# zhangganlin/vista-slam

Hardware: AMD Instinct MI355X
Metric: STA image-pairs/sec @512x384 (higher is better)
Workload: dtype f16x3-split MFMA (3 fp16 products) in the transformer and the pose head; fp16 MFMA + one block-scaled fp8 correction MFMA in the DPT head's convolutions; fp32 accumulate; 1 GPU; 512x384 batch=8 pairs/GPU STA two-view forward (BASELINE configs[1]); pairs_per_gpu=8, H=384, W=512, precision=f16x3h, parallelism=single GPU

## Files before the change

include/sta_mi355_debug.h:

```cpp
#ifndef STA_MI355_DEBUG_H
#define STA_MI355_DEBUG_H
#include "sta_mi355.h"
#ifdef __cplusplus
extern "C" {
#endif

STA_API int sta_set_gemm_variant(sta_handle* h, int variant);

STA_API int sta_debug_pick_family(int amode, int epi, long long M, int N, int K, int split, int cstride, int Ho, int Wo);

STA_API int sta_debug_gemm_plan(int amode, int epi, int M_all, int N, int K, int precision, int mx, int tail_hint, int forced_variant, int* out);

STA_API int sta_debug_last_gemm_plan(sta_handle* h, int* out);

STA_API int sta_debug_qkv_pair_plan(int precision, int M, int N_a, int N_b, int K, int mx_a, int mx_b, int tail_hint, int forced_variant, int* out);

STA_API int sta_debug_qkv_pair(sta_handle* h, const float* x_a, const float* w_a, const float* bias_a, const float* x_b,
                       const float* w_b, const float* bias_b, int S, int ntok, int K, int C, int wp,
                       float* q_a, float* k_a, float* vt_a, float* k_b, float* vt_b, void* stream);

STA_API int sta_debug_gemm(sta_handle* h, const float* A, const float* W, const float* bias, int M, int N, int K,
                   int act, int via_f16, const float* resid, float* out, void* stream);

STA_API int sta_debug_qkv_rope(sta_handle* h, const float* x, const float* W, const float* bias, int S, int ntok, int K, int C,
// ... 22 lines not shown

STA_API int sta_debug_head_final(sta_handle* h, const float* x, const float* w, const float* bias, int64_t npix,
                         float* pts, float* conf, void* stream);

STA_API int sta_debug_svd_orthogonalize(sta_handle* h, const float* m, float* r, int B, void* stream);

STA_API int sta_kernel_timing_dump(sta_handle* h, int cap, double* flops, float* ms, int* variant, int* n_out);

STA_API int sta_kernel_stamps_dump(sta_handle* h, int cap, double* out6, int* n_out);

STA_API int sta_bench_gemm_stamps(sta_handle* h, int M, int N, int K, int resid, double* out, unsigned long long* raw_host, int raw_cap, void* stream);

STA_API int sta_bench_gemm(sta_handle* h, int M, int N, int K, int iters, int tile, int ablation, float* ms_out, void* stream);
STA_API float sta_bench_gemm_last_ghz(void);
STA_API int sta_bench_attention(sta_handle* h, int S, int heads, int nq, int nk, int pose, int iters, int which, float* ms_out, void* stream);

#ifdef __cplusplus
}
#endif
#endif
```

vista_slam_amd/_lib.py:

```python
import ctypes as C
import os

PKG = os.path.dirname(os.path.abspath(__file__))
LIB_PATH = os.path.join(PKG, "libsta_mi355.so")
TEST_LIB_PATH = os.path.join(PKG, "libsta_mi355_test.so")

STA_PREC_F16 = 1
STA_PREC_F16X3 = 3
STA_PREC_F16X3H = 5
STA_PREC_F16X3M = 6
PRECISIONS = {"f16": STA_PREC_F16, "f16x3": STA_PREC_F16X3, "f16x3h": STA_PREC_F16X3H, "f16x3m": STA_PREC_F16X3M}


class StaConfig(C.Structure):
    _fields_ = [("patch_size", C.c_int32), ("enc_embed_dim", C.c_int32), ("enc_depth", C.c_int32),
                ("enc_num_heads", C.c_int32), ("dec_embed_dim", C.c_int32), ("dec_depth", C.c_int32),
                ("dec_num_heads", C.c_int32), ("mlp_ratio", C.c_int32), ("rope_base", C.c_float),
                ("ln_eps", C.c_float), ("precision", C.c_int32)]


_vp, _i, _i64, _f = C.c_void_p, C.c_int, C.c_int64, C.c_float
_fp = C.c_void_p

SIGNATURES = {
# ... 46 lines not shown
    "sta_kernel_timing_filter": (_i, [_vp, _i, _i, _i, _i, _i]),
    "sta_kernel_timing_dump_shapes": (_i, [_vp, _i, C.POINTER(_i), C.POINTER(C.c_float), C.POINTER(_i), C.POINTER(_i)]),
    "sta_range_report": (_i, [_vp, C.POINTER(C.c_ulonglong), _i]),
    "sta_last_error": (C.c_char_p, []),
    "sta_version": (C.c_char_p, []),
}

TEST_SIGNATURES = {
    "sta_set_gemm_variant": (_i, [_vp, _i]),
    "sta_kernel_timing_dump": (_i, [_vp, _i, C.POINTER(C.c_double), C.POINTER(C.c_float), C.POINTER(_i), C.POINTER(_i)]),
    "sta_kernel_stamps_dump": (_i, [_vp, _i, C.POINTER(C.c_double), C.POINTER(_i)]),
    "sta_bench_gemm_stamps": (_i, [_vp, _i, _i, _i, _i, C.POINTER(C.c_double), C.POINTER(C.c_ulonglong), _i, _vp]),
    "sta_bench_gemm": (_i, [_vp, _i, _i, _i, _i, _i, _i, C.POINTER(_f), _vp]),
    "sta_bench_gemm_last_ghz": (C.c_float, []),
    "sta_bench_attention": (_i, [_vp, _i, _i, _i, _i, _i, _i, _i, C.POINTER(_f), _vp]),
    "sta_debug_gemm": (_i, [_vp, _fp, _fp, _fp, _i, _i, _i, _i, _i, _fp, _fp, _vp]),
    "sta_debug_qkv_rope": (_i, [_vp, _fp, _fp, _fp, _i, _i, _i, _i, _i, _i, _fp, _fp, _fp, _vp]),
    "sta_debug_attention": (_i, [_vp, _fp, _fp, _fp, _i, _i, _i, _i, _i, _fp, _vp]),
    "sta_debug_attention_pose": (_i, [_vp, _fp, _fp, _fp, _i, _i, _i, _i, _fp, _vp]),
    "sta_debug_set_tail_hint": (_i, [_vp, _i]),
    "sta_debug_set_option": (_i, [_vp, _i, _i]),
    "sta_debug_pick_family": (_i, [_i, _i, C.c_longlong, _i, _i, _i, _i, _i, _i]),
    "sta_debug_gemm_plan": (_i, [_i, _i, _i, _i, _i, _i, _i, _i, _i, C.POINTER(_i)]),
    "sta_debug_last_gemm_plan": (_i, [_vp, C.POINTER(_i)]),
    "sta_debug_qkv_pair_plan": (_i, [_i, _i, _i, _i, _i, _i, _i, _i, _i, C.POINTER(_i)]),
    "sta_debug_qkv_pair": (_i, [_vp, _fp, _fp, _fp, _fp, _fp, _fp, _i, _i, _i, _i, _i, _fp, _fp, _fp, _fp, _fp, _vp]),
    "sta_debug_conv3x3": (_i, [_vp, _fp, _fp, _fp, _i, _i, _i, _i, _i, _i, _i, _i, _fp, _fp, _vp]),
    "sta_debug_convt": (_i, [_vp, _fp, _fp, _fp, _i, _i, _i, _i, _i, _fp, _vp]),
    "sta_debug_up2": (_i, [_vp, _fp, _i, _i, _i, _i, _i, _i, _fp, _vp]),
    "sta_debug_layernorm": (_i, [_vp, _fp, _fp, _fp, _i, _i, _f, _fp, _fp, _vp]),
# ... 81 lines not shown
```

vista_slam_amd/csrc/attention.h:

```cpp
#pragma once
#include "sta_common.h"
#include <type_traits>

__device__ __forceinline__ void glds16(const void* gsrc, void* lds_dst_wave_base);

struct AttnParams {
    const f16* Q_hi; const f16* Q_lo; const f16* K_hi; const f16* K_lo; const f16* Vt_hi; const f16* Vt_lo;
    f16* O_hi; f16* O_lo; int ldo;
    int S, heads, nq, nk, npad;
    int kv_shift;
    float scale_log2e;
    unsigned long long* range;
    int prefetch;
    int pose;
};

#define ATT_KV 64
#define ATT_TILE_BYTES (64 * 128)

template <bool SPLIT>
constexpr int attn_smem_bytes(int stages = 2) { return stages * (SPLIT ? 4 : 2) * ATT_TILE_BYTES; }
#define ATT_PREFETCH_TILES 4

template <bool SPLIT>
__device__ __forceinline__ void attn_pose_query(const AttnParams& p, char* smem) {
    const int tid = threadIdx.x, lane = tid & 63, wave = tid >> 6;
    const int sh = blockIdx.x;
    const int s = sh / p.heads, h = sh - s * p.heads;
    const int skv = (s + p.kv_shift) % p.S;
    const size_t qoff = ((size_t)(s * p.heads + h) * p.npad + p.nq) * 64;
// ... 57 lines not shown
#pragma unroll
            for (int e = 0; e < 8; ++e) o = __builtin_fmaf(pe[e], (float)a[u].e[e] + (SPLIT ? (float)b[u].e[e] : 0.f), o);
        }
    }
    red[8 + wave * 64 + lane] = o;
    __syncthreads();
    if (wave != 0) return;
    o = (red[8 + lane] + red[8 + 64 + lane]) + (red[8 + 128 + lane] + red[8 + 192 + lane]);
    o /= (red[4] + red[5]) + (red[6] + red[7]);
    const int64_t orow = (int64_t)p.S * p.nq + s, orows = (int64_t)p.S * p.nq + p.S;
    const size_t oo = blk_off<SPLIT>(orow, h * 64 + lane, orows);
    if (SPLIT) { f16 hh, ll; split_f16(o, hh, ll, p.range); p.O_hi[oo] = hh; p.O_hi[oo + 32] = ll; }
    else p.O_hi[oo] = to_f16_sat(o, p.range);
}

template <bool SPLIT>
__global__ __launch_bounds__(256, 2) void attn_kernel(const AttnParams p) {
    extern __shared__ __attribute__((aligned(16))) char smem[];
    constexpr int NPL = SPLIT ? 2 : 1;
    constexpr int STAGE = 2 * NPL * ATT_TILE_BYTES;
    const int npose_blocks = p.pose == 1 ? p.S * p.heads : 0;
    const int nqe = p.nq + (p.pose == 2 ? 1 : 0);
    if ((int)blockIdx.x < npose_blocks) { attn_pose_query<SPLIT>(p, smem); return; }
    const int tid = threadIdx.x, lane = tid & 63;
    const int wave = __builtin_amdgcn_readfirstlane(tid >> 6);
    const int l31 = lane & 31, lhi = lane >> 5;
    const int nqb = (nqe + 127) / 128;
    const int nwg = nqb * p.heads * p.S;
    int logical;
    {
        const int bid = blockIdx.x - npose_blocks, q = nwg / 8, r = nwg % 8, xcd = bid % 8;
        logical = (xcd < r ? xcd * (q + 1) : r * (q + 1) + (xcd - r) * q) + bid / 8;
    }
    const int qb = logical % nqb;
    const int h = (logical / nqb) % p.heads, s = logical / (nqb * p.heads);
    const int skv = (s + p.kv_shift) % p.S;
    const int q0 = qb * 128 + wave * 32;

    const size_t qoff = (size_t)(s * p.heads + h) * p.npad * 64;
    const size_t koff = (size_t)(skv * p.heads + h) * p.npad * 64;
    const size_t voff = (size_t)(skv * p.heads + h) * 64 * p.npad;

    half8 qf_hi[4], qf_lo[4];
    {
        int qrow = q0 + l31; if (qrow > nqe - 1) qrow = nqe - 1;
        const f16* qp = p.Q_hi + qoff + (size_t)qrow * 64 + lhi * 8;
#pragma unroll
        for (int kk = 0; kk < 4; ++kk) { H8 t; t.u = ldg16(qp + kk * 16); qf_hi[kk] = t.h; }
        if (SPLIT) {
            const f16* ql = p.Q_lo + qoff + (size_t)qrow * 64 + lhi * 8;
#pragma unroll
            for (int kk = 0; kk < 4; ++kk) { H8 t; t.u = ldg16(ql + kk * 16); qf_lo[kk] = t.h; }
        }
    }

    int ksrc_l[2], vsrc_l[2];
#pragma unroll
    for (int i = 0; i < 2; ++i) {
        const int row = (2 * wave + i) * 8 + (lane >> 3);
        const int sch = (lane & 7) ^ ((row >> 1) & 7);
        ksrc_l[i] = row * 64 + sch * 8;
        vsrc_l[i] = row * p.npad + sch * 8;
    }
    auto issue_tile = [&](int stage, int kv0) {
        char* sK = smem + stage * STAGE + (2 * wave) * 1024;
        char* sV = sK + NPL * ATT_TILE_BYTES;
#pragma unroll
        for (int i = 0; i < 2; ++i) {
            const size_t ko = koff + (size_t)kv0 * 64 + ksrc_l[i];
            const size_t vo = voff + (size_t)kv0 + vsrc_l[i];
            glds16(p.K_hi + ko, sK + i * 1024);
            glds16(p.Vt_hi + vo, sV + i * 1024);
            if (SPLIT) {
                glds16(p.K_lo + ko, sK + ATT_TILE_BYTES + i * 1024);
                glds16(p.Vt_lo + vo, sV + ATT_TILE_BYTES + i * 1024);
            }
        }
    };

    floatx16 oacc[2];
#pragma unroll
    for (int d = 0; d < 2; ++d)
#pragma unroll
        for (int r = 0; r < 16; ++r) oacc[d][r] = 0.f;
    float m_run = -INFINITY, l_run = 0.f;
    const bool wave_active = q0 < nqe;

    if (p.pose && wave_active) {
        float sp = 0.f;
#pragma unroll
        for (int kk = 0; kk < 4; ++kk) {
            H8 a, b; a.u = ldg16(p.K_hi + koff + (size_t)p.nk * 64 + kk * 16 + lhi * 8);
            if (SPLIT) b.u = ldg16(p.K_lo + koff + (size_t)p.nk * 64 + kk * 16 + lhi * 8);
#pragma unroll
            for (int e = 0; e < 8; ++e) {
                const float kv = (float)a.e[e] + (SPLIT ? (float)b.e[e] : 0.f);
                const float qv = (float)qf_hi[kk][e] + (SPLIT ? (float)qf_lo[kk][e] : 0.f);
                sp = __builtin_fmaf(qv, kv, sp);
            }
        }
        sp += __shfl_xor(sp, 32);
        m_run = sp * p.scale_log2e;
        l_run = lhi == 0 ? 1.f : 0.f;
#pragma unroll
        for (int d = 0; d < 2; ++d)
#pragma unroll
            for (int r = 0; r < 16; ++r) {
                const size_t o = voff + (size_t)(d * 32 + (r & 3) + 8 * (r >> 2) + 4 * lhi) * p.npad + p.nk;
                oacc[d][r] = (float)p.Vt_hi[o] + (SPLIT ? (float)p.Vt_lo[o] : 0.f);
            }
    }

    int foff_l[4];
    {
        const int swz = (l31 >> 1) & 7;
#pragma unroll
        for (int c2 = 0; c2 < 4; ++c2) foff_l[c2] = l31 * 128 + (((c2 * 2 + lhi) ^ swz) << 4);
    }

    auto tile_body = [&](auto stage_c, auto tail_c, int kv0, int stage_rt = 0) {
        constexpr int STG = decltype(stage_c)::value;
        constexpr bool TAIL = decltype(tail_c)::value;
        const char* sK = smem + STG * STAGE + stage_rt * STAGE;
        const char* sV = sK + NPL * ATT_TILE_BYTES;

        floatx16 sacc[2];
#pragma unroll
        for (int t = 0; t < 2; ++t) {
#pragma unroll
            for (int r = 0; r < 16; ++r) sacc[t][r] = 0.f;
#pragma unroll
            for (int kk = 0; kk < 4; ++kk) {
                half8 kf = *reinterpret_cast<const half8*>(sK + t * 4096 + foff_l[kk]);
                if (SPLIT) {
                    half8 kl = *reinterpret_cast<const half8*>(sK + ATT_TILE_BYTES + t * 4096 + foff_l[kk]);
                    sacc[t] = __builtin_amdgcn_mfma_f32_32x32x16_f16(kl, qf_hi[kk], sacc[t], 0, 0, 0);
                    sacc[t] = __builtin_amdgcn_mfma_f32_32x32x16_f16(kf, qf_lo[kk], sacc[t], 0, 0, 0);
                }
                sacc[t] = __builtin_amdgcn_mfma_f32_32x32x16_f16(kf, qf_hi[kk], sacc[t], 0, 0, 0);
            }
        }

        if (TAIL) {
#pragma unroll
            for (int t = 0; t < 2; ++t)
#pragma unroll
                for (int r = 0; r < 16; ++r) {
                    const int key = kv0 + t * 32 + (r & 3) + 8 * (r >> 2) + 4 * lhi;
                    if (key >= p.nk) sacc[t][r] = -INFINITY;
                }
        }
        float mx = -INFINITY;
#pragma unroll
        for (int t = 0; t < 2; ++t)
#pragma unroll
            for (int r = 0; r < 16; ++r) mx = fmaxf(mx, sacc[t][r]);
        mx = fmaxf(mx, __shfl_xor(mx, 32));
        const float m_new = fmaxf(m_run, mx * p.scale_log2e);
        const float alpha = __builtin_amdgcn_exp2f(m_run - m_new);
        const float neg_m = -m_new;
        float psum = 0.f;
#pragma unroll
        for (int t = 0; t < 2; ++t)
#pragma unroll
            for (int r = 0; r < 16; ++r) {
                const float pv = __builtin_amdgcn_exp2f(__builtin_fmaf(sacc[t][r], p.scale_log2e, neg_m));
                sacc[t][r] = pv;
                psum += pv;
            }
        l_run = l_run * alpha + psum;
        m_run = m_new;
        if (!__all(alpha == 1.0f)) {
#pragma unroll
            for (int d = 0; d < 2; ++d)
#pragma unroll
                for (int r = 0; r < 16; ++r) oacc[d][r] *= alpha;
        }

#pragma unroll
        for (int t = 0; t < 2; ++t)
#pragma unroll
            for (int w = 0; w < 2; ++w) {
                union { half8 h; unsigned u[4]; } ph, pl;
#pragma unroll
                for (int j = 0; j < 8; ++j) {
                    const float pv = sacc[t][8 * w + j];
                    const f16 hh = (f16)pv;
                    ph.h[j] = hh;
                    if (SPLIT) pl.h[j] = (f16)(pv - (float)hh);
                }
#pragma unroll
                for (int e = 0; e < 2; ++e) {
                    auto r1 = __builtin_amdgcn_permlane32_swap(ph.u[e], ph.u[2 + e], false, false);
                    ph.u[e] = r1[0]; ph.u[2 + e] = r1[1];
                    if (SPLIT) {
                        auto r2 = __builtin_amdgcn_permlane32_swap(pl.u[e], pl.u[2 + e], false, false);
                        pl.u[e] = r2[0]; pl.u[2 + e] = r2[1];
                    }
                }
                const int c2 = t * 2 + w;
#pragma unroll
                for (int d = 0; d < 2; ++d) {
                    half8 vf = *reinterpret_cast<const half8*>(sV + d * 4096 + foff_l[c2]);
                    if (SPLIT) {
                        half8 vl = *reinterpret_cast<const half8*>(sV + ATT_TILE_BYTES + d * 4096 + foff_l[c2]);
                        oacc[d] = __builtin_amdgcn_mfma_f32_32x32x16_f16(vl, ph.h, oacc[d], 0, 0, 0);
                        oacc[d] = __builtin_amdgcn_mfma_f32_32x32x16_f16(vf, pl.h, oacc[d], 0, 0, 0);
                    }
                    oacc[d] = __builtin_amdgcn_mfma_f32_32x32x16_f16(vf, ph.h, oacc[d], 0, 0, 0);
                }
            }
    };
    using std::integral_constant;
    auto step = [&](auto stage_c, auto tail_c, int it, int ntiles_) {
        constexpr int STG = decltype(stage_c)::value;
        const int kv0 = it * ATT_KV;
        if (it + 1 < ntiles_) issue_tile(STG ^ 1, kv0 + ATT_KV);
        if (wave_active) tile_body(stage_c, tail_c, kv0);
        asm volatile("s_waitcnt vmcnt(0)" ::: "memory");
        __syncthreads();
    };

    const int ntiles = (p.nk + ATT_KV - 1) / ATT_KV, nfull = p.nk / ATT_KV;
    using F = integral_constant<bool, false>; using T = integral_constant<bool, true>;
    if (p.prefetch) {
        constexpr int DMAS = 4 * NPL;
// ... 15 lines not shown
        issue_tile(0, 0);
        asm volatile("s_waitcnt vmcnt(0)" ::: "memory");
        __syncthreads();
        int it = 0;
        for (; it + 1 < nfull; it += 2) {
            step(integral_constant<int, 0>{}, F{}, it, ntiles);
            step(integral_constant<int, 1>{}, F{}, it + 1, ntiles);
        }
        if (it < nfull) { step(integral_constant<int, 0>{}, F{}, it, ntiles); ++it; }
        if (it < ntiles) {
            if (it & 1) step(integral_constant<int, 1>{}, T{}, it, ntiles);
            else step(integral_constant<int, 0>{}, T{}, it, ntiles);
        }
    }

    const float l_tot = l_run + __shfl_xor(l_run, 32);
    const float inv = 1.0f / l_tot;
    const int64_t orows = (int64_t)p.S * p.nq + (p.pose ? p.S : 0);
    if constexpr (SPLIT) {
        __syncthreads();
        char* const wl = smem + wave * (64 * 128);
        RangeAcc ra;
#pragma unroll
        for (int d = 0; d < 2; ++d) {
            const int rowb = (d * 32 + l31) * 128, sw = l31 & 7;
#pragma unroll
            for (int j = 0; j < 2; ++j) {
                union { uint4 u4; unsigned u[4]; } ch, cl;
#pragma unroll
                for (int gg = 0; gg < 2; ++gg) {
                    H4 oh, ol;
#pragma unroll
                    for (int e = 0; e < 4; ++e) split_f16(oacc[d][(2 * j + gg) * 4 + e] * inv, oh.e[e], ol.e[e], ra);
                    ch.u[2 * gg] = oh.u.x; ch.u[2 * gg + 1] = oh.u.y; cl.u[2 * gg] = ol.u.x; cl.u[2 * gg + 1] = ol.u.y;
                }
#pragma unroll
                for (int e = 0; e < 2; ++e) {
                    auto r1 = __builtin_amdgcn_permlane32_swap(ch.u[e], ch.u[2 + e], false, false);
                    ch.u[e] = r1[0]; ch.u[2 + e] = r1[1];
                    auto r2 = __builtin_amdgcn_permlane32_swap(cl.u[e], cl.u[2 + e], false, false);
                    cl.u[e] = r2[0]; cl.u[2 + e] = r2[1];
                }
                const int c = 2 * j + lhi;
                *reinterpret_cast<uint4*>(wl + rowb + ((c ^ sw) << 4)) = ch.u4;
                *reinterpret_cast<uint4*>(wl + rowb + (((4 + c) ^ sw) << 4)) = cl.u4;
            }
        }
#pragma unroll
        for (int d = 0; d < 2; ++d)
#pragma unroll
            for (int it = 0; it < 4; ++it) {
                const int qq = (lane >> 3) + 8 * it, ch = lane & 7;
                const int q = q0 + qq;
                if (q < nqe) {
                    const int64_t orow = q < p.nq ? (int64_t)s * p.nq + q : (int64_t)p.S * p.nq + s;
                    const size_t o = blk_off<true>(orow, h * 64 + d * 32, orows);
                    *reinterpret_cast<uint4*>(p.O_hi + o + ch * 8) = *reinterpret_cast<const uint4*>(wl + (d * 32 + qq) * 128 + ((ch ^ (qq & 7)) << 4));
                }
            }
    } else {
        const int q = q0 + l31;
        if (q < nqe) {
            RangeAcc ra;
            const int64_t orow = q < p.nq ? (int64_t)s * p.nq + q : (int64_t)p.S * p.nq + s;
#pragma unroll
            for (int d = 0; d < 2; ++d)
#pragma unroll
                for (int g = 0; g < 4; ++g) {
                    const int dcol = d * 32 + 8 * g + 4 * lhi;
                    const size_t o = blk_off<false>(orow, h * 64 + dcol, orows);
                    H4 oh;
#pragma unroll
                    for (int e = 0; e < 4; ++e) oh.e[e] = to_f16_sat(oacc[d][g * 4 + e] * inv, ra);
                    *reinterpret_cast<uint2*>(p.O_hi + o) = oh.u;
                }
        }
    }
}
```

vista_slam_amd/csrc/sta_bench.inc:

```

extern "C" double sta_flops_per_pair(const sta_handle* h, int H, int W) {
    if (!h) return 0;
    const sta_config& c = h->cfg;
    const double E = c.enc_embed_dim, D = c.dec_embed_dim, R = c.mlp_ratio;
    const double hp = H / 16, wp = W / 16, N = hp * wp, Np = N + 1;
    double f_enc = 2 * N * 768 * E + c.enc_depth * ((8 + 4 * R) * N * E * E + 4 * N * N * E);
    double f_dec = 4 * N * E * D + 2.0 * c.dec_depth * ((16 + 4 * R) * Np * D * D + 8 * Np * Np * D);
    auto conv = [](double hh, double ww, double ci, double co, double k) { return 2.0 * hh * ww * ci * co * k * k; };
    double h3 = floor((hp - 1) / 2) + 1, w3 = floor((wp - 1) / 2) + 1;
    double f = 0;
    f += conv(hp, wp, E, 96, 1) + 2.0 * hp * wp * 96 * 96 * 16;
    f += conv(hp, wp, D, 192, 1) + 2.0 * hp * wp * 192 * 192 * 4;
    f += conv(hp, wp, D, 384, 1);
    f += conv(hp, wp, D, 768, 1) + conv(h3, w3, 768, 768, 3);
    f += conv(4 * hp, 4 * wp, 96, 256, 3) + conv(2 * hp, 2 * wp, 192, 256, 3) + conv(hp, wp, 384, 256, 3) + conv(h3, w3, 768, 256, 3);
    f += 2 * conv(h3, w3, 256, 256, 3) + conv(hp, wp, 256, 256, 1);
    f += 4 * conv(hp, wp, 256, 256, 3) + conv(2 * hp, 2 * wp, 256, 256, 1);
    f += 4 * conv(2 * hp, 2 * wp, 256, 256, 3) + conv(4 * hp, 4 * wp, 256, 256, 1);
    f += 4 * conv(4 * hp, 4 * wp, 256, 256, 3) + conv(8 * hp, 8 * wp, 256, 256, 1);
    f += conv(8 * hp, 8 * wp, 256, 128, 3) + conv(16 * hp, 16 * wp, 128, 128, 3) + conv(16 * hp, 16 * wp, 128, 4, 1);
    double f_pose = 2.0 * (D * 512 + 2 * 512 * 512 + 512 * 13);
    return 2 * f_enc + f_dec + 2 * f + 2 * f_pose;
}

// ... 15 lines not shown
        constexpr int smem = gemm2_smem_bytes<true, BM, BN>();
        HIPCHK(hipFuncSetAttribute((const void*)gemm2_kernel<true, A_DENSE, EPI_F32, BM, BN, WMS, WNS, ABL>, hipFuncAttributeMaxDynamicSharedMemorySize, smem));
        hipLaunchKernelGGL((gemm2_kernel<true, A_DENSE, EPI_F32, BM, BN, WMS, WNS, ABL>), dim3((unsigned)(((p.M + BM - 1) / BM) * ((p.N + BN - 1) / BN))), dim3(WMS * WNS * 64), smem, st, p);
    } else {
#ifndef STA_DEV_FAST
        constexpr int smem = gemm2_smem_bytes<false, BM, BN>();
        HIPCHK(hipFuncSetAttribute((const void*)gemm2_kernel<false, A_DENSE, EPI_F32, BM, BN, WMS, WNS, ABL>, hipFuncAttributeMaxDynamicSharedMemorySize, smem));
        hipLaunchKernelGGL((gemm2_kernel<false, A_DENSE, EPI_F32, BM, BN, WMS, WNS, ABL>), dim3((unsigned)(((p.M + BM - 1) / BM) * ((p.N + BN - 1) / BN))), dim3(WMS * WNS * 64), smem, st, p);
#else
        return set_err("development build: precision f16 kernels are not compiled in");
#endif
    }
    return 0;
}

static float g_bench_ghz = 0.f;
extern "C" float sta_bench_gemm_last_ghz() { return g_bench_ghz; }

extern "C" int sta_bench_gemm(sta_handle* h, int M, int N, int K, int iters, int tile, int abl, float* ms_out, void* stream) {
    REQUIRE(h && ms_out && iters > 0, "bad argument");
    DEV_SCOPE(h->device);
    hipStream_t st = (hipStream_t)stream;
    const bool split = h->prec != STA_PREC_F16;
    int64_t bytes = ((int64_t)M * K + (int64_t)N * K) * 4 + (int64_t)M * N * 4 + N * 4 + (1 << 16);
    CHK(ensure_ws(h, bytes, st));
    h->dry = false;
    Bump ws = cur_bump(h);
    Planes A = ws.act(M, K, true);
    Lin Wt; Wt.N = N; Wt.K = K; Wt.w = ws.act(N, K, true);
    Wt.bias = (float*)ws.take((int64_t)N * 4);
    float* C = (float*)ws.take((int64_t)M * N * 4);
    unsigned long long* clk = (unsigned long long*)ws.take(16);
// ... 163 lines not shown
    return 0;
}

extern "C" int sta_bench_attention(sta_handle* h, int S, int heads, int nq, int nk, int pose, int iters, int which, float* ms_out, void* stream) {
    REQUIRE(h && ms_out && iters > 0 && S > 0 && heads > 0 && nq > 0 && nk > 0, "bad argument");
    DEV_SCOPE(h->device);
    hipStream_t st = (hipStream_t)stream;
    const bool split = h->prec != STA_PREC_F16;
    const int nmax = (nq > nk ? nq : nk) + (pose ? 1 : 0), npad = rup(nmax, 64);
    const int64_t hsz = (int64_t)S * heads * npad * 64, M = (int64_t)S * nq + (pose ? S : 0);
    CHK(ensure_ws(h, (3 * hsz + M * heads * 64) * 4 + (1 << 16), st));
    h->dry = false;
    Bump ws = cur_bump(h);
    QKVOut o; o.npad = npad; o.q = ws.planes(hsz, true); o.k = ws.planes(hsz, true); o.vt = ws.planes(hsz, true);
    Planes ao = ws.act(M, heads * 64, true);
    REQUIRE(!ws.overflow, "internal: bench workspace overflow");
    if (!split) { o.q.lo = o.k.lo = o.vt.lo = nullptr; ao.lo = nullptr; }
    hipLaunchKernelGGL(fill_rand_f16_kernel, dim3(2048), dim3(256), 0, st, o.q.hi, hsz * 2, 5u, 1.0f);
    hipLaunchKernelGGL(fill_rand_f16_kernel, dim3(2048), dim3(256), 0, st, o.k.hi, hsz * 2, 7u, 1.0f);
    hipLaunchKernelGGL(fill_rand_f16_kernel, dim3(2048), dim3(256), 0, st, o.vt.hi, hsz * 2, 9u, 1.0f);
    REQUIRE(which == 0, "sta_bench_attention: no alternative kernel in this build");
    hipEvent_t e0, e1;
    HIPCHK(hipEventCreate(&e0)); HIPCHK(hipEventCreate(&e1));
    int rc = 0;
    for (int i = 0; i < 2 && rc == 0; ++i) rc = run_attn(h, o, ao, heads * 64, S, heads, nq, nk, 0, st, pose != 0);
    HIPCHK(hipEventRecord(e0, st));
    for (int i = 0; i < iters && rc == 0; ++i) rc = run_attn(h, o, ao, heads * 64, S, heads, nq, nk, 0, st, pose != 0);
    HIPCHK(hipEventRecord(e1, st));
    if (rc != 0) return rc;
    HIPCHK(hipEventSynchronize(e1));
    float ms = 0; HIPCHK(hipEventElapsedTime(&ms, e0, e1));
    *ms_out = ms / iters;
    hipEventDestroy(e0); hipEventDestroy(e1);
    return 0;
}
#endif
```

vista_slam_amd/csrc/sta_launch.inc:

```
template <bool SPLIT, int AMODE, int EPI, int BM, int BN, int WMS, int WNS, int NSTG = 2, bool MX = false>
static int launch_gemm2(const GemmParams& p, hipStream_t st, int dev = 0) {
    static unsigned attr_done = 0;
    constexpr int smem = gemm2_smem_bytes<SPLIT, BM, BN>(NSTG);
    if (!(attr_done >> (dev & 31) & 1u)) {
        HIPCHK(hipFuncSetAttribute((const void*)gemm2_kernel<SPLIT, AMODE, EPI, BM, BN, WMS, WNS, 0, NSTG, MX>,
                                   hipFuncAttributeMaxDynamicSharedMemorySize, smem));
        attr_done |= 1u << (dev & 31);
    }
    int tm = (p.M - p.m_tail + BM - 1) / BM, tn = (p.N + BN - 1) / BN;
    const int ks = p.ksplit > 1 ? p.ksplit : 1;
    const int ntail = p.m_tail > 0 ? (p.N + 31) / 32 : 0;
    hipLaunchKernelGGL((gemm2_kernel<SPLIT, AMODE, EPI, BM, BN, WMS, WNS, 0, NSTG, MX>), dim3((unsigned)(tm * tn * ks + ntail)), dim3(WMS * WNS * 64), smem, st, p);
    return 0;
}

template <bool SPLIT, int EPI, int BM, int BN, bool MX, int WMS = 4, int WNS = 4>
static int launch_conv3h(const GemmParams& p, hipStream_t st, int dev) {
    static unsigned attr_done = 0;
    constexpr int smem = conv3h_smem_bytes<SPLIT, BM, BN>();
    static_assert(smem <= 160 * 1024, "conv3h: LDS budget");
    auto kern = conv3h_kernel<SPLIT, EPI, BM, BN, WMS, WNS, MX>;
    if (!(attr_done >> (dev & 31) & 1u)) {
        HIPCHK(hipFuncSetAttribute((const void*)kern, hipFuncAttributeMaxDynamicSharedMemorySize, smem));
        attr_done |= 1u << (dev & 31);
// ... 545 lines not shown
    HIPCHK(hipGetLastError());
    return 0;
}

static int rope_fix(sta_handle* h, const Planes& qk, int S, int heads, int npad, int ntok, hipStream_t st) {
    if (h->dry || !h->rope_foreign) return 0;
    const int64_t total = (int64_t)S * heads * (ntok + 1) * 32;
    const dim3 grid((unsigned)((total + 255) / 256));
    if (qk.lo) hipLaunchKernelGGL(rope_planes_kernel<true>, grid, dim3(256), 0, st, qk.hi, qk.lo, S, heads, npad, ntok, h->rope_pos, h->rope_tab, h->range);
    else hipLaunchKernelGGL(rope_planes_kernel<false>, grid, dim3(256), 0, st, qk.hi, qk.lo, S, heads, npad, ntok, h->rope_pos, h->rope_tab, h->range);
    HIPCHK(hipGetLastError());
    return 0;
}

static int run_attn(sta_handle* h, const QKVOut& qkv, const Planes& out, int ldo, int S, int heads,
                    int nq, int nk, int kv_shift, hipStream_t st, bool pose = false) {
    if (h->dry) return 0;
    REQUIRE(!pose || (nq == nk && nq + 1 <= qkv.npad), "internal: pose-token attention needs nq == nk < npad");
    AttnParams p; memset(&p, 0, sizeof p);
    p.range = h->range;
    p.pose = pose ? (nq % 128 != 0 ? 2 : 1) : 0;
    p.Q_hi = qkv.q.hi; p.Q_lo = qkv.q.lo; p.K_hi = qkv.k.hi; p.K_lo = qkv.k.lo; p.Vt_hi = qkv.vt.hi; p.Vt_lo = qkv.vt.lo;
    p.O_hi = out.hi; p.O_lo = out.lo; p.ldo = ldo;
    p.S = S; p.heads = heads; p.nq = nq; p.nk = nk; p.npad = qkv.npad; p.kv_shift = kv_shift;
    p.scale_log2e = 0.125f * 1.44269504088896340736f;
    const int npose = p.pose == 1 ? S * heads : 0;
    REQUIRE(!pose || (int64_t)(qkv.npad + 8 + 256) * 4 <= attn_smem_bytes<false>(), "internal: pose-query scratch exceeds the LDS allocation");
    REQUIRE(!pose || qkv.npad % 64 == 0, "internal: pose-query path needs npad % 64 == 0");
    dim3 grid((unsigned)(((nq + (p.pose == 2 ? 1 : 0) + 127) / 128) * heads * S + npose));
    p.prefetch = (nk <= ATT_PREFETCH_TILES * ATT_KV && grid.x <= 256 && h->opt[5] != 1) ? 1 : 0;
    const int stages = p.prefetch ? ATT_PREFETCH_TILES : 2;
    if (h->prec != STA_PREC_F16) {
        static unsigned attr_done = 0;
        if (!(attr_done >> (h->device & 31) & 1u)) { hipFuncSetAttribute((const void*)attn_kernel<true>, hipFuncAttributeMaxDynamicSharedMemorySize, attn_smem_bytes<true>(ATT_PREFETCH_TILES)); attr_done |= 1u << (h->device & 31); }
        hipLaunchKernelGGL(attn_kernel<true>, grid, dim3(256), attn_smem_bytes<true>(stages), st, p);
    } else {
        STA_F16ONLY(hipLaunchKernelGGL(attn_kernel<false>, grid, dim3(256), attn_smem_bytes<false>(stages), st, p));
    }
    HIPCHK(hipGetLastError());
    return 0;
// ... 48 lines not shown
```

Baseline: 195.0 pairs/s.

## Switch attention MFMA from 32x32x16 to 16x16x32 tiles with new swizzle

Rewrites the flash-attention inner loop to use 16x16x32 f16 MFMA tiles (4 key blocks x 2 query blocks per wave) instead of 32x32x16, changes the LDS swizzle pattern, and replaces shuffle-based row reductions with permlane16/32 swaps. The aim is better MFMA issue efficiency, fewer permlane shuffles when repacking P, and fewer LDS bank conflicts. It also adds a test-only cycle-counter hook and a bench helper that reports attention clock frequency. The new layout raises the MFMA instruction count per tile and changes register pressure.

```diff
diff --git a/include/sta_mi355_debug.h b/include/sta_mi355_debug.h
--- a/include/sta_mi355_debug.h
+++ b/include/sta_mi355_debug.h
@@ -60,6 +60,7 @@
 STA_API int sta_bench_gemm(sta_handle* h, int M, int N, int K, int iters, int tile, int ablation, float* ms_out, void* stream);
 STA_API float sta_bench_gemm_last_ghz(void);
 STA_API int sta_bench_attention(sta_handle* h, int S, int heads, int nq, int nk, int pose, int iters, int which, float* ms_out, void* stream);
+STA_API float sta_bench_attention_last_ghz(void);
 
 #ifdef __cplusplus
 }
diff --git a/vista_slam_amd/_lib.py b/vista_slam_amd/_lib.py
--- a/vista_slam_amd/_lib.py
+++ b/vista_slam_amd/_lib.py
@@ -84,6 +84,7 @@
     "sta_bench_gemm": (_i, [_vp, _i, _i, _i, _i, _i, _i, C.POINTER(_f), _vp]),
     "sta_bench_gemm_last_ghz": (C.c_float, []),
     "sta_bench_attention": (_i, [_vp, _i, _i, _i, _i, _i, _i, _i, C.POINTER(_f), _vp]),
+    "sta_bench_attention_last_ghz": (C.c_float, []),
     "sta_debug_gemm": (_i, [_vp, _fp, _fp, _fp, _i, _i, _i, _i, _i, _fp, _fp, _vp]),
     "sta_debug_qkv_rope": (_i, [_vp, _fp, _fp, _fp, _i, _i, _i, _i, _i, _i, _fp, _fp, _fp, _vp]),
     "sta_debug_attention": (_i, [_vp, _fp, _fp, _fp, _i, _i, _i, _i, _i, _fp, _vp]),
diff --git a/vista_slam_amd/csrc/attention.h b/vista_slam_amd/csrc/attention.h
--- a/vista_slam_amd/csrc/attention.h
+++ b/vista_slam_amd/csrc/attention.h
@@ -13,7 +13,12 @@
     unsigned long long* range;
     int prefetch;
     int pose;
+#ifdef STA_TEST_HOOKS
+    unsigned long long* clk_dbg;
+#endif
 };
+
+__device__ __forceinline__ int att_swz(int R) { return ((R >> 2) & 6) | ((R >> 1) & 1); }
 
 #define ATT_KV 64
 #define ATT_TILE_BYTES (64 * 128)
@@ -101,6 +106,23 @@
     else p.O_hi[oo] = to_f16_sat(o, p.range);
 }
 
+__device__ __forceinline__ float att_xsum16(float x) {
+    const auto r = __builtin_amdgcn_permlane16_swap(__float_as_uint(x), __float_as_uint(x), false, false);
+    return __uint_as_float(r[0]) + __uint_as_float(r[1]);
+}
+__device__ __forceinline__ float att_xsum32(float x) {
+    const auto r = __builtin_amdgcn_permlane32_swap(__float_as_uint(x), __float_as_uint(x), false, false);
+    return __uint_as_float(r[0]) + __uint_as_float(r[1]);
+}
+__device__ __forceinline__ float att_xmax16(float x) {
+    const auto r = __builtin_amdgcn_permlane16_swap(__float_as_uint(x), __float_as_uint(x), false, false);
+    return fmaxf(__uint_as_float(r[0]), __uint_as_float(r[1]));
+}
+__device__ __forceinline__ float att_xmax32(float x) {
+    const auto r = __builtin_amdgcn_permlane32_swap(__float_as_uint(x), __float_as_uint(x), false, false);
+    return fmaxf(__uint_as_float(r[0]), __uint_as_float(r[1]));
+}
+
 template <bool SPLIT>
 __global__ __launch_bounds__(256, 2) void attn_kernel(const AttnParams p) {
     extern __shared__ __attribute__((aligned(16))) char smem[];
@@ -109,9 +131,13 @@
     const int npose_blocks = p.pose == 1 ? p.S * p.heads : 0;
     const int nqe = p.nq + (p.pose == 2 ? 1 : 0);
     if ((int)blockIdx.x < npose_blocks) { attn_pose_query<SPLIT>(p, smem); return; }
+#ifdef STA_TEST_HOOKS
+    unsigned long long clk0 = 0, rt0 = 0;
+    if (p.clk_dbg) { clk0 = __builtin_readcyclecounter(); rt0 = __builtin_amdgcn_s_memrealtime(); }
+#endif
     const int tid = threadIdx.x, lane = tid & 63;
     const int wave = __builtin_amdgcn_readfirstlane(tid >> 6);
-    const int l31 = lane & 31, lhi = lane >> 5;
+    const int m16 = lane & 15, g = lane >> 4;
     const int nqb = (nqe + 127) / 128;
     const int nwg = nqb * p.heads * p.S;
     int logical;
@@ -119,25 +145,24 @@
         const int bid = blockIdx.x - npose_blocks, q = nwg / 8, r = nwg % 8, xcd = bid % 8;
         logical = (xcd < r ? xcd * (q + 1) : r * (q + 1) + (xcd - r) * q) + bid / 8;
     }
-    const int qb = logical % nqb;
+    const int qblk = logical % nqb;
     const int h = (logical / nqb) % p.heads, s = logical / (nqb * p.heads);
     const int skv = (s + p.kv_shift) % p.S;
-    const int q0 = qb * 128 + wave * 32;
+    const int q0 = qblk * 128 + wave * 32;
 
     const size_t qoff = (size_t)(s * p.heads + h) * p.npad * 64;
     const size_t koff = (size_t)(skv * p.heads + h) * p.npad * 64;
     const size_t voff = (size_t)(skv * p.heads + h) * 64 * p.npad;
 
-    half8 qf_hi[4], qf_lo[4];
-    {
-        int qrow = q0 + l31; if (qrow > nqe - 1) qrow = nqe - 1;
-        const f16* qp = p.Q_hi + qoff + (size_t)qrow * 64 + lhi * 8;
-#pragma unroll
-        for (int kk = 0; kk < 4; ++kk) { H8 t; t.u = ldg16(qp + kk * 16); qf_hi[kk] = t.h; }
-        if (SPLIT) {
-            const f16* ql = p.Q_lo + qoff + (size_t)qrow * 64 + lhi * 8;
-#pragma unroll
-            for (int kk = 0; kk < 4; ++kk) { H8 t; t.u = ldg16(ql + kk * 16); qf_lo[kk] = t.h; }
+    half8 qf_hi[2][2], qf_lo[2][2];
+#pragma unroll
+    for (int qb = 0; qb < 2; ++qb) {
+        int qrow = q0 + 16 * qb + m16; if (qrow > nqe - 1) qrow = nqe - 1;
+        const size_t qo = qoff + (size_t)qrow * 64 + g * 8;
+#pragma unroll
+        for (int ds = 0; ds < 2; ++ds) {
+            H8 t; t.u = ldg16(p.Q_hi + qo + ds * 32); qf_hi[qb][ds] = t.h;
+            if (SPLIT) { H8 u; u.u = ldg16(p.Q_lo + qo + ds * 32); qf_lo[qb][ds] = u.h; }
         }
     }
 
@@ -145,7 +170,7 @@
 #pragma unroll
     for (int i = 0; i < 2; ++i) {
         const int row = (2 * wave + i) * 8 + (lane >> 3);
-        const int sch = (lane & 7) ^ ((row >> 1) & 7);
+        const int sch = (lane & 7) ^ att_swz(row);
         ksrc_l[i] = row * 64 + sch * 8;
         vsrc_l[i] = row * p.npad + sch * 8;
     }
@@ -165,138 +190,169 @@
         }
     };
 
-    floatx16 oacc[2];
-#pragma unroll
-    for (int d = 0; d < 2; ++d)
-#pragma unroll
-        for (int r = 0; r < 16; ++r) oacc[d][r] = 0.f;
-    float m_run = -INFINITY, l_run = 0.f;
+    floatx4 oacc[4][2];
+#pragma unroll
+    for (int db = 0; db < 4; ++db)
+#pragma unroll
+        for (int qb = 0; qb < 2; ++qb)
+#pragma unroll
+            for (int i = 0; i < 4; ++i) oacc[db][qb][i] = 0.f;
+    float m_run[2] = {-INFINITY, -INFINITY}, l_run[2] = {0.f, 0.f};
     const bool wave_active = q0 < nqe;
 
     if (p.pose && wave_active) {
-        float sp = 0.f;
-#pragma unroll
-        for (int kk = 0; kk < 4; ++kk) {
-            H8 a, b; a.u = ldg16(p.K_hi + koff + (size_t)p.nk * 64 + kk * 16 + lhi * 8);
-            if (SPLIT) b.u = ldg16(p.K_lo + koff + (size_t)p.nk * 64 + kk * 16 + lhi * 8);
-#pragma unroll
-            for (int e = 0; e < 8; ++e) {
-                const float kv = (float)a.e[e] + (SPLIT ? (float)b.e[e] : 0.f);
-                const float qv = (float)qf_hi[kk][e] + (SPLIT ? (float)qf_lo[kk][e] : 0.f);
-                sp = __builtin_fmaf(qv, kv, sp);
-            }
-        }
-        sp += __shfl_xor(sp, 32);
-        m_run = sp * p.scale_log2e;
-        l_run = lhi == 0 ? 1.f : 0.f;
-#pragma unroll
-        for (int d = 0; d < 2; ++d)
-#pragma unroll
-            for (int r = 0; r < 16; ++r) {
-                const size_t o = voff + (size_t)(d * 32 + (r & 3) + 8 * (r >> 2) + 4 * lhi) * p.npad + p.nk;
-                oacc[d][r] = (float)p.Vt_hi[o] + (SPLIT ? (float)p.Vt_lo[o] : 0.f);
-            }
-    }
-
-    int foff_l[4];
+        float kp[16];
+#pragma unroll
+        for (int ds = 0; ds < 2; ++ds) {
+            H8 a, b; a.u = ldg16(p.K_hi + koff + (size_t)p.nk * 64 + ds * 32 + g * 8);
+            if (SPLIT) b.u = ldg16(p.K_lo + koff + (size_t)p.nk * 64 + ds * 32 + g * 8);
+#pragma unroll
+            for (int e = 0; e < 8; ++e) kp[ds * 8 + e] = (float)a.e[e] + (SPLIT ? (float)b.e[e] : 0.f);
+        }
+#pragma unroll
+        for (int qb = 0; qb < 2; ++qb) {
+            float sp = 0.f;
+#pragma unroll
+            for (int ds = 0; ds < 2; ++ds)
+#pragma unroll
+                for (int e = 0; e < 8; ++e) {
+                    const float qv = (float)qf_hi[qb][ds][e] + (SPLIT ? (float)qf_lo[qb][ds][e] : 0.f);
+                    sp = __builtin_fmaf(qv, kp[ds * 8 + e], sp);
+                }
+            sp = att_xsum32(att_xsum16(sp));
+            m_run[qb] = sp * p.scale_log2e;
+            l_run[qb] = g == 0 ? 1.f : 0.f;
+        }
+#pragma unroll
+        for (int db = 0; db < 4; ++db)
+#pragma unroll
+            for (int i = 0; i < 4; ++i) {
+                const size_t o = voff + (size_t)(32 * (db >> 1) + 8 * g + 4 * (db & 1) + i) * p.npad + p.nk;
+                const float v = (float)p.Vt_hi[o] + (SPLIT ? (float)p.Vt_lo[o] : 0.f);
+                oacc[db][0][i] = v; oacc[db][1][i] = v;
+            }
+    }
+
+    int foff_l[2];
     {
-        const int swz = (l31 >> 1) & 7;
-#pragma unroll
-        for (int c2 = 0; c2 < 4; ++c2) foff_l[c2] = l31 * 128 + (((c2 * 2 + lhi) ^ swz) << 4);
-    }
-
-    auto tile_body = [&](auto stage_c, auto tail_c, int kv0, int stage_rt = 0) {
+        const int R = 8 * (m16 >> 2) + (m16 & 3), swz = att_swz(R);
+#pragma unroll
+        for (int x = 0; x < 2; ++x) foff_l[x] = R * 128 + (((4 * x + g) ^ swz) << 4);
+    }
+    auto blk_b = [](int b) { return (b >> 1) * 4096 + (b & 1) * 512; };
+
+    auto tile_body = [&](auto stage_c, auto tail_c, int kv0, int stage_rt = 0) __attribute__((always_inline)) {
         constexpr int STG = decltype(stage_c)::value;
         constexpr bool TAIL = decltype(tail_c)::value;
         const char* sK = smem + STG * STAGE + stage_rt * STAGE;
         const char* sV = sK + NPL * ATT_TILE_BYTES;
 
-        floatx16 sacc[2];
-#pragma unroll
-        for (int t = 0; t < 2; ++t) {
-#pragma unroll
-            for (int r = 0; r < 16; ++r) sacc[t][r] = 0.f;
-#pragma unroll
-            for (int kk = 0; kk < 4; ++kk) {
-                half8 kf = *reinterpret_cast<const half8*>(sK + t * 4096 + foff_l[kk]);
-                if (SPLIT) {
-                    half8 kl = *reinterpret_cast<const half8*>(sK + ATT_TILE_BYTES + t * 4096 + foff_l[kk]);
-                    sacc[t] = __builtin_amdgcn_mfma_f32_32x32x16_f16(kl, qf_hi[kk], sacc[t], 0, 0, 0);
-                    sacc[t] = __builtin_amdgcn_mfma_f32_32x32x16_f16(kf, qf_lo[kk], sacc[t], 0, 0, 0);
-                }
-                sacc[t] = __builtin_amdgcn_mfma_f32_32x32x16_f16(kf, qf_hi[kk], sacc[t], 0, 0, 0);
-            }
+        floatx4 sacc[4][2];
+#pragma unroll
+        for (int kb = 0; kb < 4; ++kb)
+#pragma unroll
+            for (int qb = 0; qb < 2; ++qb)
+#pragma unroll
+                for (int i = 0; i < 4; ++i) sacc[kb][qb][i] = 0.f;
+#pragma unroll
+        for (int ds = 0; ds < 2; ++ds) {
+            half8 kf[4], kl[4];
+#pragma unroll
+            for (int kb = 0; kb < 4; ++kb) {
+                kf[kb] = *reinterpret_cast<const half8*>(sK + blk_b(kb) + foff_l[ds]);
+                if (SPLIT) kl[kb] = *reinterpret_cast<const half8*>(sK + ATT_TILE_BYTES + blk_b(kb) + foff_l[ds]);
+            }
+            if (SPLIT) {
+#pragma unroll
+                for (int kb = 0; kb < 4; ++kb)
+#pragma unroll
+                    for (int qb = 0; qb < 2; ++qb) sacc[kb][qb] = __builtin_amdgcn_mfma_f32_16x16x32_f16(kl[kb], qf_hi[qb][ds], sacc[kb][qb], 0, 0, 0);
+#pragma unroll
+                for (int kb = 0; kb < 4; ++kb)
+#pragma unroll
+                    for (int qb = 0; qb < 2; ++qb) sacc[kb][qb] = __builtin_amdgcn_mfma_f32_16x16x32_f16(kf[kb], qf_lo[qb][ds], sacc[kb][qb], 0, 0, 0);
+            }
+#pragma unroll
+            for (int kb = 0; kb < 4; ++kb)
+#pragma unroll
+                for (int qb = 0; qb < 2; ++qb) sacc[kb][qb] = __builtin_amdgcn_mfma_f32_16x16x32_f16(kf[kb], qf_hi[qb][ds], sacc[kb][qb], 0, 0, 0);
         }
 
         if (TAIL) {
 #pragma unroll
-            for (int t = 0; t < 2; ++t)
-#pragma unroll
-                for (int r = 0; r < 16; ++r) {
-                    const int key = kv0 + t * 32 + (r & 3) + 8 * (r >> 2) + 4 * lhi;
-                    if (key >= p.nk) sacc[t][r] = -INFINITY;
-                }
-        }
-        float mx = -INFINITY;
-#pragma unroll
-        for (int t = 0; t < 2; ++t)
-#pragma unroll
-            for (int r = 0; r < 16; ++r) mx = fmaxf(mx, sacc[t][r]);
-        mx = fmaxf(mx, __shfl_xor(mx, 32));
-        const float m_new = fmaxf(m_run, mx * p.scale_log2e);
-        const float alpha = __builtin_amdgcn_exp2f(m_run - m_new);
-        const float neg_m = -m_new;
-        float psum = 0.f;
-#pragma unroll
-        for (int t = 0; t < 2; ++t)
-#pragma unroll
-            for (int r = 0; r < 16; ++r) {
-                const float pv = __builtin_amdgcn_exp2f(__builtin_fmaf(sacc[t][r], p.scale_log2e, neg_m));
-                sacc[t][r] = pv;
-                psum += pv;
-            }
-        l_run = l_run * alpha + psum;
-        m_run = m_new;
-        if (!__all(alpha == 1.0f)) {
-#pragma unroll
-            for (int d = 0; d < 2; ++d)
-#pragma unroll
-                for (int r = 0; r < 16; ++r) oacc[d][r] *= alpha;
-        }
-
-#pragma unroll
-        for (int t = 0; t < 2; ++t)
-#pragma unroll
-            for (int w = 0; w < 2; ++w) {
-                union { half8 h; unsigned u[4]; } ph, pl;
+            for (int kb = 0; kb < 4; ++kb)
+#pragma unroll
+                for (int i = 0; i < 4; ++i) {
+                    const int key = kv0 + 32 * (kb >> 1) + 8 * g + 4 * (kb & 1) + i;
+                    if (key >= p.nk) { sacc[kb][0][i] = -INFINITY; sacc[kb][1][i] = -INFINITY; }
+                }
+        }
+        float alpha[2];
+#pragma unroll
+        for (int qb = 0; qb < 2; ++qb) {
+            float mx = -INFINITY;
+#pragma unroll
+            for (int kb = 0; kb < 4; ++kb)
+#pragma unroll
+                for (int i = 0; i < 4; ++i) mx = fmaxf(mx, sacc[kb][qb][i]);
+            mx = att_xmax32(att_xmax16(mx));
+            const float m_new = fmaxf(m_run[qb], mx * p.scale_log2e);
+            alpha[qb] = __builtin_amdgcn_exp2f(m_run[qb] - m_new);
+            const float neg_m = -m_new;
+            float psum = 0.f;
+#pragma unroll
+            for (int kb = 0; kb < 4; ++kb)
+#pragma unroll
+                for (int i = 0; i < 4; ++i) {
+                    const float pv = __builtin_amdgcn_exp2f(__builtin_fmaf(sacc[kb][qb][i], p.scale_log2e, neg_m));
+                    sacc[kb][qb][i] = pv;
+                    psum += pv;
+                }
+            l_run[qb] = l_run[qb] * alpha[qb] + psum;
+            m_run[qb] = m_new;
+        }
+        if (!__all(alpha[0] == 1.0f && alpha[1] == 1.0f)) {
+#pragma unroll
+            for (int db = 0; db < 4; ++db)
+#pragma unroll
+                for (int qb = 0; qb < 2; ++qb)
+#pragma unroll
+                    for (int i = 0; i < 4; ++i) oacc[db][qb][i] *= alpha[qb];
+        }
+
+#pragma unroll
+        for (int sl = 0; sl < 2; ++sl) {
+            half8 ph[2], pl[2];
+#pragma unroll
+            for (int qb = 0; qb < 2; ++qb)
 #pragma unroll
                 for (int j = 0; j < 8; ++j) {
-                    const float pv = sacc[t][8 * w + j];
+                    const float pv = sacc[2 * sl + (j >> 2)][qb][j & 3];
                     const f16 hh = (f16)pv;
-                    ph.h[j] = hh;
-                    if (SPLIT) pl.h[j] = (f16)(pv - (float)hh);
-                }
-#pragma unroll
-                for (int e = 0; e < 2; ++e) {
-                    auto r1 = __builtin_amdgcn_permlane32_swap(ph.u[e], ph.u[2 + e], false, false);
-                    ph.u[e] = r1[0]; ph.u[2 + e] = r1[1];
-                    if (SPLIT) {
-                        auto r2 = __builtin_amdgcn_permlane32_swap(pl.u[e], pl.u[2 + e], false, false);
-                        pl.u[e] = r2[0]; pl.u[2 + e] = r2[1];
-                    }
-                }
-                const int c2 = t * 2 + w;
-#pragma unroll
-                for (int d = 0; d < 2; ++d) {
-                    half8 vf = *reinterpret_cast<const half8*>(sV + d * 4096 + foff_l[c2]);
-                    if (SPLIT) {
-                        half8 vl = *reinterpret_cast<const half8*>(sV + ATT_TILE_BYTES + d * 4096 + foff_l[c2]);
-                        oacc[d] = __builtin_amdgcn_mfma_f32_32x32x16_f16(vl, ph.h, oacc[d], 0, 0, 0);
-                        oacc[d] = __builtin_amdgcn_mfma_f32_32x32x16_f16(vf, pl.h, oacc[d], 0, 0, 0);
-                    }
-                    oacc[d] = __builtin_amdgcn_mfma_f32_32x32x16_f16(vf, ph.h, oacc[d], 0, 0, 0);
-                }
-            }
+                    ph[qb][j] = hh;
+                    if (SPLIT) pl[qb][j] = (f16)(pv - (float)hh);
+                }
+            half8 vf[4], vl[4];
+#pragma unroll
+            for (int db = 0; db < 4; ++db) {
+                vf[db] = *reinterpret_cast<const half8*>(sV + blk_b(db) + foff_l[sl]);
+                if (SPLIT) vl[db] = *reinterpret_cast<const half8*>(sV + ATT_TILE_BYTES + blk_b(db) + foff_l[sl]);
+            }
+            if (SPLIT) {
+#pragma unroll
+                for (int db = 0; db < 4; ++db)
+#pragma unroll
+                    for (int qb = 0; qb < 2; ++qb) oacc[db][qb] = __builtin_amdgcn_mfma_f32_16x16x32_f16(vl[db], ph[qb], oacc[db][qb], 0, 0, 0);
+#pragma unroll
+                for (int db = 0; db < 4; ++db)
+#pragma unroll
+                    for (int qb = 0; qb < 2; ++qb) oacc[db][qb] = __builtin_amdgcn_mfma_f32_16x16x32_f16(vf[db], pl[qb], oacc[db][qb], 0, 0, 0);
+            }
+#pragma unroll
+            for (int db = 0; db < 4; ++db)
+#pragma unroll
+                for (int qb = 0; qb < 2; ++qb) oacc[db][qb] = __builtin_amdgcn_mfma_f32_16x16x32_f16(vf[db], ph[qb], oacc[db][qb], 0, 0, 0);
+        }
     };
     using std::integral_constant;
     auto step = [&](auto stage_c, auto tail_c, int it, int ntiles_) {
@@ -342,66 +398,59 @@
         }
     }
 
-    const float l_tot = l_run + __shfl_xor(l_run, 32);
-    const float inv = 1.0f / l_tot;
+    float inv[2];
+#pragma unroll
+    for (int qb = 0; qb < 2; ++qb) inv[qb] = 1.0f / att_xsum32(att_xsum16(l_run[qb]));
     const int64_t orows = (int64_t)p.S * p.nq + (p.pose ? p.S : 0);
     if constexpr (SPLIT) {
         __syncthreads();
         char* const wl = smem + wave * (64 * 128);
         RangeAcc ra;
 #pragma unroll
-        for (int d = 0; d < 2; ++d) {
-            const int rowb = (d * 32 + l31) * 128, sw = l31 & 7;
+        for (int qb = 0; qb < 2; ++qb)
 #pragma unroll
             for (int j = 0; j < 2; ++j) {
-                union { uint4 u4; unsigned u[4]; } ch, cl;
-#pragma unroll
-                for (int gg = 0; gg < 2; ++gg) {
-                    H4 oh, ol;
-#pragma unroll
-                    for (int e = 0; e < 4; ++e) split_f16(oacc[d][(2 * j + gg) * 4 + e] * inv, oh.e[e], ol.e[e], ra);
-                    ch.u[2 * gg] = oh.u.x; ch.u[2 * gg + 1] = oh.u.y; cl.u[2 * gg] = ol.u.x; cl.u[2 * gg + 1] = ol.u.y;
-                }
-#pragma unroll
-                for (int e = 0; e < 2; ++e) {
-                    auto r1 = __builtin_amdgcn_permlane32_swap(ch.u[e], ch.u[2 + e], false, false);
-                    ch.u[e] = r1[0]; ch.u[2 + e] = r1[1];
-                    auto r2 = __builtin_amdgcn_permlane32_swap(cl.u[e], cl.u[2 + e], false, false);
-                    cl.u[e] = r2[0]; cl.u[2 + e] = r2[1];
-                }
-                const int c = 2 * j + lhi;
-                *reinterpret_cast<uint4*>(wl + rowb + ((c ^ sw) << 4)) = ch.u4;
-                *reinterpret_cast<uint4*>(wl + rowb + (((4 + c) ^ sw) << 4)) = cl.u4;
-            }
-        }
-#pragma unroll
-        for (int d = 0; d < 2; ++d)
+                H8 ch, cl;
+#pragma unroll
+                for (int e = 0; e < 8; ++e) split_f16(oacc[2 * j + (e >> 2)][qb][e & 3] * inv[qb], ch.e[e], cl.e[e], ra);
+                const int R = j * 32 + qb * 16 + m16, sw = R & 7;
+                *reinterpret_cast<uint4*>(wl + R * 128 + ((g ^ sw) << 4)) = ch.u;
+                *reinterpret_cast<uint4*>(wl + R * 128 + (((4 + g) ^ sw) << 4)) = cl.u;
+            }
+#pragma unroll
+        for (int j = 0; j < 2; ++j)
 #pragma unroll
             for (int it = 0; it < 4; ++it) {
                 const int qq = (lane >> 3) + 8 * it, ch = lane & 7;
                 const int q = q0 + qq;
                 if (q < nqe) {
                     const int64_t orow = q < p.nq ? (int64_t)s * p.nq + q : (int64_t)p.S * p.nq + s;
-                    const size_t o = blk_off<true>(orow, h * 64 + d * 32, orows);
-                    *reinterpret_cast<uint4*>(p.O_hi + o + ch * 8) = *reinterpret_cast<const uint4*>(wl + (d * 32 + qq) * 128 + ((ch ^ (qq & 7)) << 4));
+                    const size_t o = blk_off<true>(orow, h * 64 + j * 32, orows);
+                    *reinterpret_cast<uint4*>(p.O_hi + o + ch * 8) = *reinterpret_cast<const uint4*>(wl + (j * 32 + qq) * 128 + ((ch ^ (qq & 7)) << 4));
                 }
             }
     } else {
-        const int q = q0 + l31;
-        if (q < nqe) {
-            RangeAcc ra;
-            const int64_t orow = q < p.nq ? (int64_t)s * p.nq + q : (int64_t)p.S * p.nq + s;
-#pragma unroll
-            for (int d = 0; d < 2; ++d)
-#pragma unroll
-                for (int g = 0; g < 4; ++g) {
-                    const int dcol = d * 32 + 8 * g + 4 * lhi;
-                    const size_t o = blk_off<false>(orow, h * 64 + dcol, orows);
-                    H4 oh;
-#pragma unroll
-                    for (int e = 0; e < 4; ++e) oh.e[e] = to_f16_sat(oacc[d][g * 4 + e] * inv, ra);
-                    *reinterpret_cast<uint2*>(p.O_hi + o) = oh.u;
-                }
-        }
-    }
-}
+        RangeAcc ra;
+#pragma unroll
+        for (int qb = 0; qb < 2; ++qb) {
+            const int q = q0 + qb * 16 + m16;
+            if (q < nqe) {
+                const int64_t orow = q < p.nq ? (int64_t)s * p.nq + q : (int64_t)p.S * p.nq + s;
+#pragma unroll
+                for (int j = 0; j < 2; ++j) {
+                    const size_t o = blk_off<false>(orow, h * 64 + j * 32 + 8 * g, orows);
+                    H8 oh;
+#pragma unroll
+                    for (int e = 0; e < 8; ++e) oh.e[e] = to_f16_sat(oacc[2 * j + (e >> 2)][qb][e & 3] * inv[qb], ra);
+                    *reinterpret_cast<uint4*>(p.O_hi + o) = oh.u;
+                }
+            }
+        }
+    }
+#ifdef STA_TEST_HOOKS
+    if (p.clk_dbg && tid == 0 && (blockIdx.x & 63) == 0) {
+        atomicAdd(p.clk_dbg, __builtin_readcyclecounter() - clk0);
+        atomicAdd(p.clk_dbg + 1, __builtin_amdgcn_s_memrealtime() - rt0);
+    }
+#endif
+}
diff --git a/vista_slam_amd/csrc/sta_bench.inc b/vista_slam_amd/csrc/sta_bench.inc
--- a/vista_slam_amd/csrc/sta_bench.inc
+++ b/vista_slam_amd/csrc/sta_bench.inc
@@ -53,8 +53,9 @@
     return 0;
 }
 
-static float g_bench_ghz = 0.f;
+static float g_bench_ghz = 0.f, g_bench_attn_ghz = 0.f;
 extern "C" float sta_bench_gemm_last_ghz() { return g_bench_ghz; }
+extern "C" float sta_bench_attention_last_ghz() { return g_bench_attn_ghz; }
 
 extern "C" int sta_bench_gemm(sta_handle* h, int M, int N, int K, int iters, int tile, int abl, float* ms_out, void* stream) {
     REQUIRE(h && ms_out && iters > 0, "bad argument");
@@ -248,6 +249,7 @@
     Bump ws = cur_bump(h);
     QKVOut o; o.npad = npad; o.q = ws.planes(hsz, true); o.k = ws.planes(hsz, true); o.vt = ws.planes(hsz, true);
     Planes ao = ws.act(M, heads * 64, true);
+    unsigned long long* clk = (unsigned long long*)ws.take(16);
     REQUIRE(!ws.overflow, "internal: bench workspace overflow");
     if (!split) { o.q.lo = o.k.lo = o.vt.lo = nullptr; ao.lo = nullptr; }
     hipLaunchKernelGGL(fill_rand_f16_kernel, dim3(2048), dim3(256), 0, st, o.q.hi, hsz * 2, 5u, 1.0f);
@@ -266,6 +268,12 @@
     float ms = 0; HIPCHK(hipEventElapsedTime(&ms, e0, e1));
     *ms_out = ms / iters;
     hipEventDestroy(e0); hipEventDestroy(e1);
-    return 0;
-}
-#endif
+    HIPCHK(hipMemsetAsync(clk, 0, 16, st));
+    for (int i = 0; i < 3; ++i) CHK(run_attn(h, o, ao, heads * 64, S, heads, nq, nk, 0, st, pose != 0, clk));
+    unsigned long long hc[2] = {0, 0};
+    HIPCHK(hipMemcpyAsync(hc, clk, 16, hipMemcpyDeviceToHost, st));
+    HIPCHK(hipStreamSynchronize(st));
+    g_bench_attn_ghz = hc[1] ? (float)((double)hc[0] / ((double)hc[1] / 100e6) * 1e-9) : 0.f;
+    return 0;
+}
+#endif
diff --git a/vista_slam_amd/csrc/sta_launch.inc b/vista_slam_amd/csrc/sta_launch.inc
--- a/vista_slam_amd/csrc/sta_launch.inc
+++ b/vista_slam_amd/csrc/sta_launch.inc
@@ -583,7 +583,7 @@
 }
 
 static int run_attn(sta_handle* h, const QKVOut& qkv, const Planes& out, int ldo, int S, int heads,
-                    int nq, int nk, int kv_shift, hipStream_t st, bool pose = false) {
+                    int nq, int nk, int kv_shift, hipStream_t st, bool pose = false, unsigned long long* clk = nullptr) {
     if (h->dry) return 0;
     REQUIRE(!pose || (nq == nk && nq + 1 <= qkv.npad), "internal: pose-token attention needs nq == nk < npad");
     AttnParams p; memset(&p, 0, sizeof p);
@@ -593,6 +593,11 @@
     p.O_hi = out.hi; p.O_lo = out.lo; p.ldo = ldo;
     p.S = S; p.heads = heads; p.nq = nq; p.nk = nk; p.npad = qkv.npad; p.kv_shift = kv_shift;
     p.scale_log2e = 0.125f * 1.44269504088896340736f;
+#ifdef STA_TEST_HOOKS
+    p.clk_dbg = clk;
+#else
+    (void)clk;
+#endif
     const int npose = p.pose == 1 ? S * heads : 0;
     REQUIRE(!pose || (int64_t)(qkv.npad + 8 + 256) * 4 <= attn_smem_bytes<false>(), "internal: pose-query scratch exceeds the LDS allocation");
     REQUIRE(!pose || qkv.npad % 64 == 0, "internal: pose-query path needs npad % 64 == 0");
```

Result: no change. 195.5 pairs/s, median of 6 (+0.3%).
